# allentran/golds-rl-gym

Hardware: AMD Instinct MI355X
Metric: env-steps/sec (whole node), 32k parallel Swarm-v0 envs, 20-step PAAC rollout (higher is better)
Workload: dtype f32; 1 GPU; Swarm-v0 84x84, 32768 envs per GPU, T=20 PAAC update, conv policy of train_paac_conv.py (BASELINE configs[2]); envs_per_gpu=32768, envs_total=32768, rollout_steps=20, policy=conv, train=True, swarm_math=exact, env_state_dtype=f64, streams=4, gradient_exchange=none

## Files before the change

### golds-rl-gym_amd/csrc/net_conv.hip

```cpp
#include <stdlib.h>
#include <string.h>

#include <chrono>
#include <cmath>
#include <string>
#include <vector>

#include "../../include/goldsrl_net.h"
#include "common.h"
#include "net_gemm.h"
#include "net_paac_host.h"
#include "net_reduce.inc"
#include "rng.h"

namespace grl {

enum : uint32_t { RS_ACTION = 16 };

struct ConvOffsets {
    static constexpr long c1w = 0, c1b = c1w + 8 * 8 * 3 * 32, c2w = c1b + 32, c2b = c2w + 4 * 4 * 32 * 64, c3w = c2b + 64,
                          c3b = c3w + 3 * 3 * 64 * 64, d1w = c3b + 64, d1b = d1w + 3136 * 512, d2w = d1b + 512,
                          d2b = d2w + 512 * 256, p1w = d2b + 256, p1b = p1w + 256 * 512, heads = p1b + 512;
};
constexpr int GRL_MAX_ACTIONS = 4;
// ... 71 lines not shown
    unsigned long long *ws_m2s;
    signed char *ws_ulist;
    void *ws_idx[24];
    bool train_ready;
};

struct NetEval {
    double *rewards, *normals;
    int32_t *length;
    uint8_t *finished, *alive;
    float *envact, *actions;
    float *tr_mu, *tr_sigma, *tr_raw, *tr_value;
    size_t cap_steps, cap_norm, cap_envs, cap_act, cap_trace;
    int max_steps, trace_env, keep_actions;
    bool unchecked;
    int flag_before;
};

struct grl_net : NetLane, grl::PaacCommNet {
    grl_net_config cfg;
    int chunk;
    float *paramsT;
    float *w3t, *w2t;
    float *w3f;
    float *wpvT;
    int shared_trunk;
    double sfrac;
    double pfrac[3];
    float *tbgimg, *tbgz, *tbgimg3, *tbgz3, *tybg;
    int *tbglist;
    int obs_index;
    int trunk_skip;
    int patch_skip;
    int gemm_f32, range_fallback_on, range_fallbacks, range_bits_last, update_skipped_last;
    int f32_by_fallback, f32_clean_passes, range_return_k, range_returns;
    float absmax_last;
    int loss_scale_on;
    int acc1;
    int expand3_gather;
    int expand2_gemm, ctiles;
    float *w2corr;
    grl::HeadOff ho;
    int npad, ptiles, pslices, pslice_rows, pwgrad_xcd, pdgrad_xcd, pwgrad_pair, pdgrad_pair, swgrad_pair, swgrad_chunks, slots_xcd;
    int tn_wgs, tn_wgs_dense;
    size_t slab_floats, slab_used, slabb_floats, slabb_used;
    std::vector<grl::RJob> rq;
    std::vector<int> rq_dst;
    int T, B;
    uint8_t *ro_lb, *ro_ab, *ro_pos, *ro_done;
    float *ro_act, *ro_envact, *ro_val, *ro_rew, *ro_y, *ro_adv, *ro_boot, *ro_pmu, *ro_psg;
    float *mu, *sigma, *vs;
    uint8_t *tmp_lb, *tmp_ab, *tmp_pos;
    int tmp_envs;
    bool prof_on;
    std::vector<hipEvent_t> prof_ev;
    std::vector<unsigned char> prof_tag;
    std::vector<double> prof_launch_flops;
    int prof_tag_cur;
    size_t prof_used;
    double prof_flops;
    int last_n;
    long ht_rollouts, ht_updates;
    double ht_rollout_ms, ht_train_enq_ms, ht_train_wait_ms;
    double ht_train_t0;
    int keep_level;
    float *keep;
// ... 277 lines not shown
        for (int d = 1; d < 32; d <<= 1) {
            const int o = __shfl_up(incl, d, 32);
            if (co >= d) incl += o;
        }
        const int total = __shfl(incl, 31, 32);
        int at = incl - n;
#pragma unroll
        for (int j = 0; j < 4; ++j) {
            const unsigned int k = (w >> (8 * j)) & 255u;
            if (k) ev[at++] = (unsigned short)((((ky * 8 + half * 4 + j) * 2 + c) << 7) | k);
        }
        float acc = b1[co];
        for (int e = 0; e < total; ++e) {
            const int code = ev[e];
            acc += vtab[(code >> 7) & 1][code & 127] * wl[(code >> 7) * 32 + co];
        }
        if (live) sraw[(size_t)env * 12800 + pix * 32 + co] = acc;
    }
    __syncthreads();
    if (tid < 90 && bx != 255) {
        const int idx = bx * G + by;
        cnt[tid < 80 ? 0 : 1][idx >> 2] = 0u;
    }
  }
}

__device__ __forceinline__ float wave_sum(float v) {
#pragma unroll
    for (int o = 32; o > 0; o >>= 1) v += __shfl_xor(v, o);
    return v;
}

constexpr int kHeadRows = 4;
template <int A>
__global__ __launch_bounds__(256) void heads_forward_kernel(const float *__restrict__ p1, const float *__restrict__ v2,
                                                            const float *__restrict__ params, HeadOff o, int n, float scale,
                                                            float *__restrict__ mu, float *__restrict__ sigma, float *__restrict__ vs) {
    const int row0 = (blockIdx.x * 4 + (threadIdx.x >> 6)) * kHeadRows, lane = threadIdx.x & 63;
    if (row0 >= n) return;
    const float *muw = params + o.muw, *sgw = params + o.sgw, *v3w = params + o.v3w;
    float wm[8][A], ws[8][A];
#pragma unroll
    for (int j = 0; j < 8; ++j) {
        const int k = (j >> 2) * 256 + 4 * lane + (j & 3);
#pragma unroll
        for (int a = 0; a < A; ++a) { wm[j][a] = muw[k * A + a]; ws[j][a] = sgw[k * A + a]; }
    }
    const float4 wv = make_float4(v3w[4 * lane], v3w[4 * lane + 1], v3w[4 * lane + 2], v3w[4 * lane + 3]);
    float4 x0[kHeadRows], x1[kHeadRows], xv[kHeadRows];
#pragma unroll
    for (int r = 0; r < kHeadRows; ++r) {
        const size_t row = (size_t)min(row0 + r, n - 1);
        x0[r] = reinterpret_cast<const float4 *>(p1 + row * 512)[lane];
        x1[r] = reinterpret_cast<const float4 *>(p1 + row * 512 + 256)[lane];
        xv[r] = reinterpret_cast<const float4 *>(v2 + row * 256)[lane];
    }
    float mine = 0.f;
#pragma unroll
    for (int r = 0; r < kHeadRows; ++r) {
        const float x[8] = {x0[r].x, x0[r].y, x0[r].z, x0[r].w, x1[r].x, x1[r].y, x1[r].z, x1[r].w};
#pragma unroll
        for (int a = 0; a < A; ++a) {
            float m = 0.f, sg = 0.f;
#pragma unroll
            for (int j = 0; j < 8; ++j) { m += x[j] * wm[j][a]; sg += x[j] * ws[j][a]; }
            m = wave_sum(m);
            sg = wave_sum(sg);
            if (lane == 16 * r + a) mine = m;
            if (lane == 16 * r + A + a) mine = sg;
        }
        const float zv = wave_sum(xv[r].x * wv.x + xv[r].y * wv.y + xv[r].z * wv.z + xv[r].w * wv.w);
        if (lane == 16 * r + 2 * A) mine = zv;
    }
    const int r = lane >> 4, i = lane & 15, row = row0 + r;
    if (row >= n || i > 2 * A) return;
    if (i < A) {
        mu[(size_t)row * A + i] = tanhf(mine + params[o.mub + i]);
    } else if (i < 2 * A) {
        sigma[(size_t)row * A + (i - A)] = 1.0f / (1.0f + expf(-(mine + params[o.sgb + (i - A)])));
    } else {
        const float zv = mine + params[o.v3b];
        const float sp = zv > 20.f ? zv : log1pf(expf(zv));
        vs[row] = -scale * sp;
    }
}
#define GRL_HEADS_DISPATCH(A_, CALL)                                  \
    switch (A_) {                                                     \
        case 1: { constexpr int kA = 1; CALL; } break;                \
        case 2: { constexpr int kA = 2; CALL; } break;                \
        case 3: { constexpr int kA = 3; CALL; } break;                \
        default: { constexpr int kA = 4; CALL; } break;               \
    }

struct ObsRecord {
    const uint32_t *lb, *ab, *pos;
    uint32_t *ro_lb, *ro_ab, *ro_pos;
    int nenv;
    int32_t *done_count;
};
__global__ void sample_actions_kernel(const float *__restrict__ mu, const float *__restrict__ sigma, int i0, int n, uint64_t seed,
                                      uint32_t env_off, uint32_t counter, float *__restrict__ raw, float *__restrict__ envact, ObsRecord R) {
    int i = blockIdx.x * blockDim.x + threadIdx.x;
    if (R.done_count && i == 0) *R.done_count = 0;
    for (int w = i; w < R.nenv * 50; w += gridDim.x * blockDim.x) {
        if (w < R.nenv * 40) R.ro_lb[w] = R.lb[w];
        else if (w < R.nenv * 45) R.ro_ab[w - R.nenv * 40] = R.ab[w - R.nenv * 40];
        else R.ro_pos[w - R.nenv * 45] = R.pos[w - R.nenv * 45];
    }
// ... 56 lines not shown
    if (net->shared_trunk) {
        net->a3sh = b; b += (c / 10) * 3136;
        net->d3 = b; b += c * 1600;
        net->m3 = reinterpret_cast<unsigned long long *>(b); b += c * 50;
    } else {
        net->a3 = b; b += c * 3136;
    }
    net->d1 = b; b += c * 512;
    net->d2 = b; b += c * 256;
    net->p1 = b; b += c * 512;
    net->v1 = b; b += c * 512;
    net->v2 = b; b += c * 256;
    net->mb_d2 = reinterpret_cast<unsigned long long *>(b); net->mb_v1 = net->mb_d2 + c * 4; b += c * 32;
    if (net->shared_trunk && net->keep_level >= 2) {
        net->sraw = b; b += (c / 10) * 12800;
        net->a2sh = b; b += (c / 10) * 5184;
        net->d2s = b; b += c * 576;
        net->m2s = reinterpret_cast<unsigned long long *>(b); b += c * 18;
        net->ulist = reinterpret_cast<signed char *>(b); b += ((c * 9 + 3) / 4 + 3) / 4 * 4;
    }
    size_t walked = (size_t)(b - b0) * sizeof(float);
    if (net->shared_trunk && net->keep_level >= 3) {
        const size_t used = (size_t)(b - b0);
        char *q = reinterpret_cast<char *>(b + (((used + 31) & ~(size_t)31) - used));
#define X(m, bytes) net->m = reinterpret_cast<decltype(net->m)>(q); q += ((size_t)(bytes) + 127) & ~(size_t)127;
        GRL_IDX_LIST(X)
#undef X
        walked = (size_t)(q - reinterpret_cast<char *>(b0));
    }
    return walked;
}

static int forward_chunk(grl_net *net, const uint8_t *lb, const uint8_t *ab, const uint8_t *pos, int nenv, float *mu,
                         float *sigma, float *vs, bool reuse_tail = false, bool skip_heads = false) {
    hipStream_t st = net->h->stream;
    const float *P = net->params, *PT = net->paramsT;
    const int n = nenv * 10;
    net->last_n = n;
    net->pitem_on_side = 0;
    if (net->shared_trunk) {
        int rc;
        if (reuse_tail && net->keep_level >= 3) {
            if ((rc = slot_prof(net, n))) return rc;
            rc = patch_prof(net);
        } else if (reuse_tail && net->keep_level >= 2) {
            if ((rc = slot_index(net, pos, n))) return rc;
            if (net->trunk_skip && net->expand2_gemm && (rc = trunk_index(net, lb, ab, pos, nenv))) return rc;
            rc = patch_sort(net, n);
        } else {
            rc = forward_conv12_shared(net, lb, ab, pos, nenv, !reuse_tail);
        }
        if (rc) return rc;
    } else {
    net->prof_tag_cur = PT_PER_AGENT;
    hipLaunchKernelGGL(conv1_sparse_kernel, dim3(nenv), dim3(256), 0, st, lb, ab, pos, P + ConvOffsets::c1w, P + ConvOffsets::c1b,
                       net->a1, net->h->cfg.grid_size, (float *)nullptr);
    {
        GatherConv2 g{net->a1, n * 81};
        EpiBiasAct e{net->a2, 64, P + ConvOffsets::c2b, ACT_RELU};
        GemmTimer t(net, 2.0 * n * 81 * 512 * 64);
        launch_rowk<256, 64, kW256M, kW256N, GatherConv2, EpiBiasAct>(net, dim3(1, (n * 81 + 255) / 256), st, g, PT + ConvOffsets::c2w, 512, 64, e);
    }
    }
    if (!reuse_tail) {
    if (net->shared_trunk) {
        if (int rc = forward_conv3_dense1_shared(net, nenv, pos)) return rc;
    } else {
        GatherConv3 g{net->a2, n * 49};
        EpiBiasAct e{net->a3, 64, P + ConvOffsets::c3b, ACT_RELU};
        GemmTimer t(net, 2.0 * n * 49 * 576 * 64);
        launch_rowk<256, 64, kW256M, kW256N, GatherConv3, EpiBiasAct>(net, dim3(1, (n * 49 + 255) / 256), st, g, PT + ConvOffsets::c3w, 576, 64, e);
    }
    net->prof_tag_cur = net->shared_trunk ? PT_DENSE_FWD : PT_PER_AGENT;
    auto dense = [&](const float *in, int K, const float *w, const float *b, int N, float *out, unsigned long long *bits) {
        DenseRows g{in, n, K, K};
        GemmTimer t(net, 2.0 * n * K * N);
        if (bits) {
            EpiBiasActBits e{out, N, b, bits, N >> 6};
            launch_rowk<128, 128, kW128M, kW128N, DenseRows, EpiBiasActBits>(net, dim3(N / 128, (n + 127) / 128), st, g, w, K, N, e);
        } else {
            EpiBiasAct e{out, N, b, ACT_RELU};
            launch_rowk<128, 128, kW128M, kW128N, DenseRows, EpiBiasAct>(net, dim3(N / 128, (n + 127) / 128), st, g, w, K, N, e);
        }
    };
    if (!net->shared_trunk) dense(net->a3, 3136, PT + ConvOffsets::d1w, P + ConvOffsets::d1b, 512, net->d1, nullptr);
    dense(net->d1, 512, PT + ConvOffsets::d2w, P + ConvOffsets::d2b, 256, net->d2, net->mb_d2);
    {
        DenseRows g{net->d2, n, 256, 256};
        GemmTimer t(net, 2.0 * n * 256 * 1024);
        EpiBiasActSplit e{net->p1, net->v1, 512, 512, P + ConvOffsets::p1b, P + net->ho.v1b, net->mb_v1, 8};
        launch_rowk<128, 128, kW128M, kW128N, DenseRows, EpiBiasActSplit, true, true, 1, true>(net, dim3(1024 / 128, (n + 127) / 128), st, g, net->wpvT, 256, 1024, e);
    }
    dense(net->v1, 512, PT + net->ho.v2w, P + net->ho.v2b, 256, net->v2, nullptr);
    }
    if (!skip_heads)
    GRL_HEADS_DISPATCH(net->ho.A, hipLaunchKernelGGL(heads_forward_kernel<kA>, dim3((n + 4 * kHeadRows - 1) / (4 * kHeadRows)), dim3(256), 0, st, net->p1, net->v2, P, net->ho, n,
                                                      net->cfg.scale, mu, sigma, vs));
    PAAC_HIP(net, hipGetLastError());
    return GRL_OK;
}

static int forward_all(grl_net *net, const uint8_t *lb, const uint8_t *ab, const uint8_t *pos, int n_envs, float *mu, float *sigma,
                       float *vs, long slot0 = -1) {
    const int ce = net->chunk / 10;
    int rc = lanes_fork(net);
    if (rc) return rc;
    const int nl = lanes_active(net);
    for (int e0 = 0; e0 < n_envs; e0 += ce) {
        int ne = n_envs - e0 < ce ? n_envs - e0 : ce;
        use_lane(net, (e0 / ce) % nl);
        net->last_lane = net->cur_lane;
        bind_activations(net, slot0 < 0 ? -1 : slot0 + e0 / ce);
        rc = forward_chunk(net, lb + (size_t)e0 * 160, ab + (size_t)e0 * 20, pos + (size_t)e0 * 20, ne,
                           mu + (size_t)e0 * 10 * net->ho.A, sigma + (size_t)e0 * 10 * net->ho.A, vs + (size_t)e0 * 10);
        if (rc) { (void)lanes_join(net); return rc; }
    }
    return lanes_join(net);
}

static int alloc_lane_forward(grl_net *n) {
    const size_t c = n->chunk;
    int rc = GRL_OK;
    auto A = [&](float **p, size_t cnt) { if (rc == GRL_OK) rc = paac_alloc(n, p, cnt); };
    A(&n->grads, n->ho.total);
    const size_t gather_ws = (size_t)n->ctiles * 256 * 576 + (c * 25 + 256) * 4 + (c * 25 + 1024) + 2 * ((c + 255) / 256 + 1) * 64 + 4096;
    A(&n->a2, std::max(c * 5184, gather_ws)); A(&n->d1, c * 512); A(&n->d2, c * 256); A(&n->p1, c * 512); A(&n->v1, c * 512); A(&n->v2, c * 256);
    if (!n->shared_trunk) { A(&n->a1, c * 12800); A(&n->a3, c * 3136); }
    A(&n->sraw, (c / 10) * 12800); A(&n->z2sh, (c / 10) * 5184);
    A(&n->a2sh, (c / 10) * 5184); A(&n->d2s, c * 9 * 64); if (rc == GRL_OK) rc = paac_alloc(n, &n->m2s, c * 9); A(&n->z3sh, (c / 10) * 3136);
// ... 172 lines not shown
    grl_net *n = new grl_net();
    n->h = h; n->cfg = *cfg; n->chunk = cfg->max_chunk_samples; n->alloc_waits = true;
    n->ho = head_offsets(cfg->num_actions); n->num_params = n->ho.total;
    n->T = 0; n->B = 0; n->tmp_envs = 0; n->prof_on = false; n->prof_used = 0; n->prof_flops = 0; n->last_n = 0; n->prof_tag_cur = 0;
    n->ro_lb = nullptr; n->slab_floats = 0; n->slab_used = 0; n->slabb_floats = 0; n->slabb_used = 0; n->w3t = n->w2t = nullptr;
    n->mu = n->sigma = n->vs = nullptr;
    n->keep_level = 0;
    n->ht_rollouts = n->ht_updates = 0; n->ht_rollout_ms = n->ht_train_enq_ms = n->ht_train_wait_ms = 0.0; n->ht_train_t0 = 0.0;
    n->keep = nullptr; n->keep_slots = 0; n->param_version = 0; n->keep_version = -1;
    n->keep_max_level = 3; n->keep_free_capped = false; n->keep_free_cap = 0; n->keep_headroom = 0; n->keep_free_seen = 0;
    n->resident_last = 0;
    if (const char *e = getenv("GRL_NET_KEEP_LEVEL")) n->keep_max_level = atoi(e);
    n->keep_free_capped = free_capped; n->keep_free_cap = (size_t)free_mb << 20;
    n->shared_trunk = (cfg->reserved & GRL_NET_F_PER_AGENT_TRUNK) ? 0 : 1;
    n->cur_lane = 0; n->last_lane = 0;
    for (int k = 0; k < GRL_MAX_LANES; ++k) { n->lane_stream[k] = nullptr; n->ev_join[k] = nullptr; n->side_stream[k] = nullptr; n->ev_side0[k] = n->ev_side1[k] = n->ev_side2[k] = nullptr; }
    n->idx_side = 0; n->side_now = 0; n->pitem_on_side = 0;
    n->lane_stream[0] = h->stream; n->ev_fork = nullptr; n->nlanes = 1;
    const size_t c = n->chunk;
    n->ptiles = (int)((c + 255) / 256) + 9;
    n->ctiles = (int)((c + 255) / 256) + 4;
    {
        const char *lsk = getenv("GRL_NET_LOSS_SCALE");
        n->loss_scale_on = (lsk && strcmp(lsk, "off") == 0) ? 0 : 1;
        const char *gm = getenv("GRL_NET_GEMM"), *rf = getenv("GRL_NET_RANGE_FALLBACK");
        n->gemm_f32 = (gm && strcmp(gm, "f32") == 0) ? 1 : 0;
        n->range_fallback_on = (rf && strcmp(rf, "off") == 0) ? 0 : 1;
        n->range_fallbacks = 0; n->range_bits_last = 0; n->update_skipped_last = 0;
        n->f32_by_fallback = 0; n->f32_clean_passes = 0; n->range_returns = 0; n->absmax_last = 0.f;
        n->range_return_k = 4;
        if (const char *rr = getenv("GRL_NET_RANGE_RETURN")) n->range_return_k = strcmp(rr, "off") == 0 ? 0 : std::max(0, atoi(rr));
        const char *psk = getenv("GRL_PATCH_SKIP");
        n->patch_skip = (psk && strcmp(psk, "off") == 0) ? 0 : 1;
        const char *oix = getenv("GRL_OBS_INDEX");
        n->obs_index = (oix && strcmp(oix, "off") == 0) ? 0 : 1;
        const char *tsk = getenv("GRL_TRUNK_SKIP");
        n->trunk_skip = (tsk && strcmp(tsk, "off") == 0) ? 0 : 1;
        n->pfrac[0] = n->pfrac[1] = n->pfrac[2] = 1.0; n->sfrac = 1.0;
        const char *e2 = getenv("GRL_NET_EXPAND2");
        n->expand2_gemm = (e2 && strcmp(e2, "lds") == 0) ? 0 : 1;
        { const char *e3 = getenv("GRL_NET_EXPAND3"); n->expand3_gather = (e3 && strcmp(e3, "prod") == 0) ? 0 : 1;
          const char *a1 = getenv("GRL_NET_ACC1"); n->acc1 = (a1 && strcmp(a1, "off") == 0) ? 0 : 1; }
    }
    n->pslice_rows = PATCH_SLICE_ROWS; n->pwgrad_xcd = 1;
    if (const char *e = getenv("GRL_PATCH_SLICE")) { const int v = atoi(e); if (v == 256 || v == 512 || v == 1024 || v == 2048 || v == 4096 || v == 8192) n->pslice_rows = v; }
    if (const char *e = getenv("GRL_PATCH_WGRAD_XCD")) n->pwgrad_xcd = atoi(e);
    n->pwgrad_pair = 1;
    if (const char *e = getenv("GRL_PATCH_WGRAD_PAIR")) n->pwgrad_pair = strcmp(e, "off") != 0 && strcmp(e, "0") != 0;
    n->pdgrad_pair = 1;
    if (const char *e = getenv("GRL_PATCH_DGRAD_PAIR")) n->pdgrad_pair = strcmp(e, "off") != 0 && strcmp(e, "0") != 0;
    n->swgrad_pair = 1;
    if (const char *e = getenv("GRL_SLOT_WGRAD_PAIR")) n->swgrad_pair = strcmp(e, "off") != 0 && strcmp(e, "0") != 0;
    n->slots_xcd = 1;
    if (const char *e = getenv("GRL_SLOTS_XCD")) n->slots_xcd = strcmp(e, "off") != 0 && strcmp(e, "0") != 0;
    n->swgrad_chunks = 0;
    if (const char *e = getenv("GRL_SLOT_WGRAD_CHUNKS")) n->swgrad_chunks = std::max(0, atoi(e));
    n->pdgrad_xcd = 1;
    n->tn_wgs = 1024; n->tn_wgs_dense = 512;
    if (const char *e = getenv("GRL_TN_WGS")) { const int v = atoi(e); if (v >= 256 && v <= 4096) n->tn_wgs = v; }
    if (const char *e = getenv("GRL_TN_WGS_DENSE")) { const int v = atoi(e); if (v >= 128 && v <= 4096) n->tn_wgs_dense = v; }
    if (const char *e = getenv("GRL_PATCH_DGRAD_XCD")) n->pdgrad_xcd = atoi(e) != 0;
    n->pslices = (int)((c + n->pslice_rows - 1) / n->pslice_rows) + 9;
    n->npad = (int)((c + 255) / 256 * 256);
    int rc = GRL_OK;
    auto A = [&](float **p, size_t cnt) { if (rc == GRL_OK) rc = paac_alloc(n, p, cnt); };
    A(&n->params, n->ho.total); A(&n->paramsT, n->ho.total); A(&n->adam_m, n->ho.total); A(&n->adam_v, n->ho.total);
// ... 392 lines not shown
```

### golds-rl-gym_amd/csrc/net_gemm.h

```cpp
#pragma once
#include <hip/hip_runtime.h>
#include <stdint.h>

#include <type_traits>
#include <utility>

namespace grl {

template <class E, class = void>
struct epi_row_bits : std::false_type {};
template <class E>
struct epi_row_bits<E, std::void_t<decltype(E::kRowBits)>> : std::bool_constant<E::kRowBits> {};

template <class E, class = void>
struct epi_row_auxn : std::false_type {};
template <class E>
struct epi_row_auxn<E, std::void_t<decltype(E::kRowAuxN)>> : std::bool_constant<E::kRowAuxN> {};
template <class E, class = void>
struct epi_add_aux : std::false_type {};
template <class E>
struct epi_add_aux<E, std::void_t<decltype(E::kAddAux)>> : std::bool_constant<E::kAddAux> {};

typedef float f32x16 __attribute__((ext_vector_type(16)));
typedef float f32x4 __attribute__((ext_vector_type(4)));
// ... 192 lines not shown
        off = (long)r * ld;
        iy0 = ix0 = 0;
    }
    __device__ __forceinline__ void tap(int k0, int &toff, int &ty, int &tx) const {
        toff = k0;
        ty = tx = 0;
    }
    __device__ __forceinline__ bool ok(int, int, int, int) const { return true; }
    __device__ __forceinline__ bool tile_ok(int, int) const { return true; }
    __device__ __forceinline__ bool tile_active(int m0) const { return !rows_dev || m0 < *rows_dev; }
    __device__ __forceinline__ int bk(int k0, int) const { return k0; }
    __device__ __forceinline__ int bn(int n0, int) const { return n0; }
    __device__ __forceinline__ int2 ahandle(int m) const { return make_int2(m, 0); }
    __device__ __forceinline__ bool hvalid(int2) const { return true; }
    __device__ __forceinline__ int bhandle(int m) const { return m; }
    __device__ __forceinline__ void rowh(int2 h, long &off, int &iy0, int &ix0) const { row(h.x, off, iy0, ix0); }
    __device__ __forceinline__ void mrange(int z, int mc, int &mbeg, int &mend) const { mbeg = z * mc; mend = min(rows, mbeg + mc); }
};

struct DenseRowsKU : DenseRows {
    static constexpr int kMaxK = 64 * 64;
    const unsigned *u;
    __device__ __forceinline__ unsigned long long wg_ctx(int) const { return (unsigned long long)u[0] | ((unsigned long long)u[1] << 32); }
    __device__ __forceinline__ bool tile_ok_c(unsigned long long c, int k0) const { return (c >> (k0 >> 6)) & 1ull; }
    __device__ __forceinline__ int bk_c(unsigned long long, int k0) const { return k0; }
};
struct DenseRowsNU : DenseRows {
    const unsigned *u;
    __device__ __forceinline__ bool n_ok(int, int n0) const { return (u[n0 >> 11] >> ((n0 >> 6) & 31)) & 1u; }
};
struct DenseRowsIU : DenseRows {
    const unsigned *u;
    __device__ __forceinline__ bool i_ok(int, int i0) const { return (u[i0 >> 11] >> ((i0 >> 6) & 31)) & 1u; }
};

struct DenseRowsGroups {
    static constexpr bool kRelu = false;
    const float *base;
    int rows, ld, k, npad, nlive, bnstep, cpc;
    __device__ __forceinline__ int K() const { return k; }
    __device__ __forceinline__ void row(int r, long &off, int &iy0, int &ix0) const {
        off = (long)r * ld;
        iy0 = ix0 = 0;
    }
    __device__ __forceinline__ void tap(int k0, int &toff, int &ty, int &tx) const {
        toff = k0;
        ty = tx = 0;
    }
    __device__ __forceinline__ bool ok(int, int, int, int) const { return true; }
    __device__ __forceinline__ bool tile_ok(int, int) const { return true; }
    __device__ __forceinline__ bool tile_active(int m0) const { return m0 % npad < nlive; }
    __device__ __forceinline__ int bk(int k0, int) const { return k0; }
    __device__ __forceinline__ int bn(int n0, int m0) const { return n0 + (m0 / npad) * bnstep; }
    __device__ __forceinline__ int2 ahandle(int m) const { return make_int2(m, 0); }
    __device__ __forceinline__ bool hvalid(int2) const { return true; }
    __device__ __forceinline__ int bhandle(int m) const { return m; }
    __device__ __forceinline__ void rowh(int2 h, long &off, int &iy0, int &ix0) const { row(h.x, off, iy0, ix0); }
    __device__ __forceinline__ void mrange(int z, int mc, int &mbeg, int &mend) const {
        const int g = z / cpc, c = z - g * cpc;
        mbeg = g * npad + c * mc;
        mend = min(g * npad + nlive, mbeg + mc);
    }
};

struct T2SlotGather {
    static constexpr bool kRelu = false;
// ... 630 lines not shown
        b0[b] = *reinterpret_cast<const float4 *>(Bf + f32_off(brow + b * 16, 8 * kg));
        b1[b] = *reinterpret_cast<const float4 *>(Bf + f32_off(brow + b * 16, 8 * kg + 4));
    }
#define GRL_F32_STEP(AV, BV)                                                                                          \
    _Pragma("unroll") for (int a = 0; a < TM; ++a)                                                                    \
        _Pragma("unroll") for (int b = 0; b < TN; ++b) acc[a][b] = __builtin_amdgcn_mfma_f32_16x16x4f32(AV, BV, acc[a][b], 0, 0, 0);
    GRL_F32_STEP(a0[a].x, b0[b].x) GRL_F32_STEP(a0[a].y, b0[b].y) GRL_F32_STEP(a0[a].z, b0[b].z) GRL_F32_STEP(a0[a].w, b0[b].w)
    GRL_F32_STEP(a1[a].x, b1[b].x) GRL_F32_STEP(a1[a].y, b1[b].y) GRL_F32_STEP(a1[a].z, b1[b].z) GRL_F32_STEP(a1[a].w, b1[b].w)
#undef GRL_F32_STEP
}

template <class T, class = void> struct ag_has_ctx : std::false_type {};
template <class T> struct ag_has_ctx<T, std::void_t<decltype(std::declval<const T &>().wg_ctx(0))>> : std::true_type {};
template <class AG> __device__ __forceinline__ auto ag_ctx(const AG &ag, int m0) {
    if constexpr (ag_has_ctx<AG>::value) return ag.wg_ctx(m0);
    else return m0;
}
template <class AG, class C> __device__ __forceinline__ bool ag_tile_ok(const AG &ag, const C &c, int m0, int k0) {
    if constexpr (ag_has_ctx<AG>::value) return ag.tile_ok_c(c, k0);
    else return ag.tile_ok(m0, k0);
}
template <class AG, class C> __device__ __forceinline__ int ag_bk(const AG &ag, const C &c, int m0, int k0) {
    if constexpr (ag_has_ctx<AG>::value) return ag.bk_c(c, k0);
    else return ag.bk(k0, m0);
}
template <class T, class = void> struct ag_has_n_ok : std::false_type {};
template <class T> struct ag_has_n_ok<T, std::void_t<decltype(std::declval<const T &>().n_ok(0, 0))>> : std::true_type {};
template <class T, class = void> struct ag_has_i_ok : std::false_type {};
template <class T> struct ag_has_i_ok<T, std::void_t<decltype(std::declval<const T &>().i_ok(0, 0))>> : std::true_type {};
template <class T, class = void> struct ag_pair_n : std::false_type {};
template <class T> struct ag_pair_n<T, std::void_t<decltype(T::kPairN)>> : std::bool_constant<T::kPairN> {};
template <class T, class = void> struct ag_pair_i : std::false_type {};
template <class T> struct ag_pair_i<T, std::void_t<decltype(T::kPairI)>> : std::bool_constant<T::kPairI> {};

template <int BM, int BN, int WGM, int WGN, class AG, class Epi, int XCD_ORDER = 1, bool FENCE = true, bool F32 = false, int NBUF = 1, bool ACC1 = false>
__global__ __launch_bounds__(64 * WGM * WGN, ACC1 ? (WGM * WGN == 8 ? 6 : 4) : WGM * WGN / 2) void gemm_rowk(AG ag, const float *__restrict__ Bt, int ldb, int N, Epi epi) {
    constexpr int BK = 32, LDH = kLdh, NT = 64 * WGM * WGN, RPP = NT / 8;
    constexpr int WM = BM / WGM, WN = BN / WGN, TM = WM / 16, TN = WN / 16;
    constexpr int NA = BM / RPP;
    constexpr int NB = BN / RPP;
    static_assert((WGM * WGN == 4 || WGM * WGN == 8) && TM >= 1 && TN >= 1 && NA >= 1 && BN % RPP == 0, "4 or 8 waves");
    static_assert(NBUF == 1 || NBUF == 2, "one or two LDS buffers");
    __shared__ __attribute__((aligned(16))) unsigned short As[NBUF][2][BM * LDH];
    static_assert(!(ACC1 && F32), "the fp32 form has one accumulator set anyway");
    __shared__ __attribute__((aligned(16))) unsigned short Bs[NBUF][ACC1 ? 3 : 2][BN * LDH];

    const int tid = threadIdx.x, lane = tid & 63, wave = tid >> 6;
    const int wm = wave / WGN, wn = wave - wm * WGN;
    int bx = blockIdx.x, by = blockIdx.y;
    if constexpr (XCD_ORDER == 2) {
        const int nt = (ag.live_rows() + BM - 1) / BM, tpx = (nt + 7) >> 3, w = blockIdx.y;
        if ((w >> 3) >= tpx) return;
        by = (w & 7) * tpx + (w >> 3);
        if (by >= nt) return;
    }
    if (XCD_ORDER == 1) {
        const int nx = gridDim.x, L = by * nx + bx, g = L / (8 * nx);
        if ((g + 1) * 8 <= (int)gridDim.y) {
            const int l = L - g * 8 * nx;
            by = g * 8 + (l & 7);
            bx = l >> 3;
        }
    }
    const int m0 = by * BM, n0 = bx * BN;
    if (!ag.tile_active(m0)) return;
    constexpr bool PAIRN = ag_pair_n<AG>::value;
// ... 242 lines not shown
            for (int a = 0; a < TM; ++a)
#pragma unroll
                for (int r = 0; r < 4; ++r)
                    if (erow + a * 16 + r < M) sum += epi.value(acc[a][b][r], eax[a][b][r]);
            sum += __shfl_xor(sum, 16);
            sum += __shfl_xor(sum, 32);
            const int col = ecol + b * 16;
            if (kg == 0 && col < N) epi.csum[(long)(by * WGM + wm) * N + col] = sum;
        }
    }
    if constexpr (epi_row_bits<Epi>::value) {
        static_assert(WN == 64, "a wave covers exactly one 64-column block");
#pragma unroll
        for (int a = 0; a < TM; ++a)
#pragma unroll
            for (int r = 0; r < 4; ++r) {
                unsigned long long w = 0ull;
#pragma unroll
                for (int b = 0; b < TN; ++b) {
                    const unsigned long long bal = __ballot(epi.bit(acc[a][b][r], eax[a][b][r]));
                    w |= ((bal >> (16 * kg)) & 0xFFFFull) << (16 * b);
                }
                const int row = erow + a * 16 + r;
                if (l16 == 0 && row < M) epi.store_bits(row, ecolbase, w, rax[a][r]);
            }
    }
#undef GRL_LOAD_TILE
#undef GRL_STORE_TILE
#undef GRL_STORE_PLANES
#undef GRL_STORE_PLANES_B
}

template <int BM, int BN, int WGM, int WGN, class AG, int XCD_ORDER = 1, bool F32 = false>
__global__ __launch_bounds__(64 * WGM * WGN, WGM * WGN / 2) void gemm_tn(AG ag, const float *__restrict__ dY, int J, int mc, float *__restrict__ slab) {
    constexpr int BK = 32, LDH = kLdh, NT = 64 * WGM * WGN;
    constexpr int WM = BM / WGM, WN = BN / WGN, TM = WM / 16, TN = WN / 16;
    constexpr int A4 = BM / 4, B4 = BN / 4;
    constexpr int NA = BK * A4 / NT, NB = BK * B4 / NT;
    static_assert((WGM * WGN == 4 || WGM * WGN == 8) && NA >= 1 && NB >= 1 && NA <= 4 && NB <= 4 && (NA != 3) && (NB != 3), "tile size");
    __shared__ __attribute__((aligned(16))) unsigned short As[2][BM * LDH];
    __shared__ __attribute__((aligned(16))) unsigned short Bs[2][BN * LDH];
    const int tid = threadIdx.x, lane = tid & 63, wave = tid >> 6;
    const int wm = wave / WGN, wn = wave - wm * WGN;
    int bx = blockIdx.x, by = blockIdx.y, bz = blockIdx.z;
    if (XCD_ORDER == 2) {
        const int nx = gridDim.x, ny = gridDim.y, l = by * nx + bx, g = l / (8 * ny);
        if ((g + 1) * 8 <= nx) {
            const int r = l - g * 8 * ny;
            bx = g * 8 + (r & 7);
            by = r >> 3;
        } else {
            const int r = l - g * 8 * ny, w = nx - g * 8;
            by = r / w;
            bx = g * 8 + (r - by * w);
        }
    }
    if (XCD_ORDER == 1) {
        const int nx = gridDim.x, T = nx * gridDim.y, L = bz * T + by * nx + bx, g = L / (8 * T);
        if ((g + 1) * 8 <= (int)gridDim.z) {
            const int l = L - g * 8 * T, t = l >> 3;
            bz = g * 8 + (l & 7);
            by = t / nx;
            bx = t - by * nx;
        }
    }
    constexpr bool PAIR = ag_pair_i<AG>::value;
    const int i0 = bx * BM, j0 = by * BN;
    const int I = ag.K();
    int mbeg, mend;
    ag.mrange(bz, mc, mbeg, mend);
    int2 pp = make_int2(0, 0);
    if constexpr (PAIR) {
        static_assert(!PAIR || BM == 128, "two 64-column halves");
        pp = ag.pair(bz, bx);
        if (pp.x < 0) return;
    } else if constexpr (ag_has_i_ok<AG>::value) {
        if (!ag.i_ok(bz, i0)) return;
    }

    int toff, ty, tx;
    ag.tap(PAIR ? (((int)(threadIdx.x % (BM / 4)) < 16 ? pp.x : max(pp.y, 0)) * 64) : i0, toff, ty, tx);

    const int ca = tid % A4, cb = tid % B4;
    int ga = tid / A4, gb = tid / B4;
    if (NA == 4) ga ^= (ca >> 1) & 1;
    if (NA == 2) ga ^= ((ca >> 1) & 1) << 1;
    if (NB == 4) gb ^= (cb >> 1) & 1;
    if (NB == 2) gb ^= ((cb >> 1) & 1) << 1;
    if (NB == 1) gb ^= ((cb >> 1) & 1) << 2;
    const int ma = NA * ga, mb = NB * gb;
    const int acol = PAIR ? toff + (ca & 15) * 4 : toff + ca * 4;
    const bool ahalf_ok = !PAIR || ca < 16 || pp.y >= 0;
    float4 ra[NA], rb[NB];
    unsigned vma = 0, vmb = 0;
    int2 ia[NA];
    int ib[NB];
    unsigned iva = 0;
#define GRL_LOAD_IDX(mt_)                                                                                          \
    {                                                                                                              \
        _Pragma("unroll") for (int i = 0; i < NA; ++i) {                                                           \
// ... 239 lines not shown
```

### golds-rl-gym_amd/csrc/net_slab_plan.h

```cpp
#pragma once
#include <stddef.h>

namespace grl {

struct SlabPlan {
    int chunks;
    int mc;
};

inline SlabPlan slab_plan(int wg_target, int tiles, int min_chunks, int rows, size_t floats_per_chunk, size_t slab_floats) {
    int chunks = (wg_target + tiles - 1) / tiles;
    if (min_chunks > chunks) chunks = min_chunks;
    if (chunks > 1024) chunks = 1024;
    if ((size_t)chunks * floats_per_chunk > slab_floats) chunks = (int)(slab_floats / floats_per_chunk);
    if (chunks < 1 || rows == 0) return {chunks, 0};
    const int mc = ((rows + chunks - 1) / chunks + 31) / 32 * 32;
    return {(rows + mc - 1) / mc, mc};
}

}
```

### golds-rl-gym_amd/csrc/net_train.inc

```

#include "net_slab_plan.h"

namespace grl {

static inline double host_now_ms() {
    return std::chrono::duration<double, std::milli>(std::chrono::steady_clock::now().time_since_epoch()).count();
}

static int rq_flush(grl_net *net) {
    const int nj = (int)net->rq.size();
    if (!nj) { net->slab_used = 0; net->slabb_used = 0; return GRL_OK; }
    std::vector<int> phase(nj, 0);
    int maxph = 0;
    for (int k = 0; k < nj; ++k) {
        for (int i = 0; i < k; ++i) phase[k] += net->rq_dst[i] == net->rq_dst[k];
        maxph = std::max(maxph, phase[k]);
    }
    for (int ph = 0; ph <= maxph; ++ph) {
        int k = 0;
        while (k < nj) {
            RBatch B;
            B.njobs = 0;
            int blocks = 0;
            for (; k < nj && B.njobs < kRJobs; ++k) {
// ... 892 lines not shown
    }
    return GRL_OK;
}

static int bwd_conv2_dgrad(const BwdCtx &c) {
    const auto [net, st, P, Gr, n, nenv, trunk] = c;
    net->prof_tag_cur = PT_ENV_DGRAD;
    float *cs5 = slabb_take(net, ((size_t)nenv * 100 / 128 + 2) * kW128M * 128);
    if (!cs5) return paac_fail(net, GRL_E_INVALID, "backward_chunk: column-sum buffer too small");
    if (trunk) {
        rowk_launch<128, 128, 2, 2, false>(net, GatherT2Rows{net->dz2, net->tblklist, net->trows_n + 1, nenv * 100}, net->w2t, 256, 128,
                                    EpiGradStride2Rows{net->gt, net->sraw, cs5, P + ConvOffsets::c1b, net->tblklist, net->trows_n + 1},
                                    2.0 * trunk_live(net, 1, (double)nenv * 100) * 256 * 128);
        hipLaunchKernelGGL(fold_class_sums_kernel, dim3(kFoldParts), dim3(256), 0, st, cs5, (nenv * 100 + 127) / 128 * 2, net->cfold,
                           (const int *)(net->trows_n + 1));
    } else {
        rowk_launch<128, 128, 2, 2, false>(net, GatherT2{net->dz2, nenv * 100}, net->w2t, 256, 128,
                                    EpiGradStride2<true, true>{net->gt, net->sraw, cs5}, 2.0 * nenv * 100 * 256 * 128);
        hipLaunchKernelGGL(fold_class_sums_kernel, dim3(kFoldParts), dim3(256), 0, st, cs5, (nenv * 100 + 127) / 128 * 2, net->cfold,
                           (const int *)nullptr);
    }
    {
        RJob j{};
        j.kind = RJ_FOLDFINAL; j.blocks = 1; j.p0 = net->cfold; j.d0 = Gr + ConvOffsets::c1b;
        rq_push(net, RD_C1B, j);
    }
    return GRL_OK;
}

static int bwd_dense_wgrad(const BwdCtx &c) {
    const auto [net, st, P, Gr, n, nenv, trunk] = c;
    int rc;
    if ((rc = tn_launch<128, 128, 2, 2>(net, RD_V2W, DenseRows{net->v1, n, 512, 512}, 512, net->gv2, 256, Gr + net->ho.v2w, 1, 0.0, 0, net->tn_wgs_dense))) return rc;
    if ((rc = tn_launch<128, 128, 2, 2>(net, RD_V1W, DenseRows{net->d2, n, 256, 256}, 256, net->gv1, 512, Gr + net->ho.v1w, 1, 0.0, 0, net->tn_wgs_dense))) return rc;
    if ((rc = tn_launch<128, 128, 2, 2>(net, RD_P1W, DenseRows{net->d2, n, 256, 256}, 256, net->gp1, 512, Gr + ConvOffsets::p1w, 1, 0.0, 0, net->tn_wgs_dense))) return rc;
    if ((rc = tn_launch<128, 128, 2, 2>(net, RD_D2W, DenseRows{net->d1, n, 512, 512}, 512, net->gd2, 256, Gr + ConvOffsets::d2w, 1, 0.0, 0, net->tn_wgs_dense))) return rc;
    return GRL_OK;
}

static int bwd_dense1_wgrad(const BwdCtx &c) {
    const auto [net, st, P, Gr, n, nenv, trunk] = c;
    int rc;
    net->prof_tag_cur = PT_ENV_WGRAD;
    if (trunk) {
        constexpr int I = 3136, J = 512;
        int chunks, mc;
        float *slab = slab_plan_take(net, net->tn_wgs, (I / 64) * (J / 128), 0, nenv, (size_t)I * J, "dense1 per-env weight gradient: slab too small", &chunks, &mc);
        if (!slab) return GRL_E_INVALID;
        {
            GemmTimer t(net, 2.0 * nenv * 64.0 * trunk_union_pixels(net) * J);
            launch_tn<64, 128, 2, 2, DenseRowsIU>(net, dim3(I / 64, J / 128, chunks), st, DenseRowsIU{{net->a3sh, nenv, 3136, 3136}, net->tumask},
                                                  net->gd1sh, J, mc, slab);
        }
        RJob j{};
        j.kind = RJ_UMASK; j.blocks = (int)(((long)I * J + 255) / 256); j.i0 = chunks; j.n = (long)I * J; j.p0 = slab; j.p1 = net->tumask;
        j.p2 = net->tbgz3 + 64; j.p3 = net->tug; j.d0 = Gr + ConvOffsets::d1w;
        rq_push(net, RD_D1W, j);
    } else if ((rc = tn_launch<64, 128, 2, 2>(net, RD_D1W, DenseRows{net->a3sh, nenv, 3136, 3136}, 3136, net->gd1sh, 512, Gr + ConvOffsets::d1w))) return rc;
    {
        float *pslab = slab_take(net, (size_t)net->pslices * 1600 * 512);
        if (!pslab) return paac_fail(net, GRL_E_INVALID, "backward_chunk: slab too small for the patch slices");
        PatchRows g{net->d3, net->perm, net->tilegroup, net->ptiles * 256, 1600, 1600, 0, net->sbeg, net->send, net->patch_skip ? net->tmask : nullptr,
                    net->patch_skip ? net->zmask : nullptr};
        {
            net->prof_tag_cur = PT_PATCH_WGRAD;
            GemmTimer t(net, 2.0 * n * 1600 * 512 * net->pfrac[2]);
            if (net->pwgrad_pair) {
                PatchRowsPair gp{g};
// ... 347 lines not shown
}

using namespace grl;

extern "C" {

int grl_net_rollout(grl_net *net, int32_t T, int32_t reward_layout) {
    if (!net || T <= 0 || T > 1024 || (reward_layout != 0 && reward_layout != 1)) return paac_fail(net, GRL_E_INVALID, "grl_net_rollout: bad argument");
    const double ht0 = host_now_ms();
    grl_handle *h = net->h;
    if (net->ho.A != 2) return paac_fail(net, GRL_E_INVALID, "grl_net_rollout: SwarmEnv.step takes (10, 2) actions; this net was built with num_actions != 2");
    hipSetDevice(h->cfg.device_id);
    int rc = ensure_rollout_bufs(net, T);
    if (rc) return rc;
    const int E = h->E, B = E * 10, ce = net->chunk / 10, nchunks = (E + ce - 1) / ce;
    net->T = T;
    net->keep_version = net->keep && (size_t)T * nchunks <= net->keep_slots ? net->param_version : -1;
    if (reward_layout == 1) PAAC_HIP(net, hipMemsetAsync(net->ro_rew, 0, (size_t)T * B * 4, h->stream));
    if ((rc = lanes_fork(net))) return rc;
    const int nl = lanes_active(net);
    net->side_now = nchunks == 1;
    struct SideOff { grl_net *n; ~SideOff() { n->side_now = 0; } } side_off{net};
    const unsigned long counter0 = net->act_counter;
    net->act_counter += (unsigned long)T;
    for (int t = 0; t <= T; ++t)
        for (int c = 0; c < nchunks; ++c) {
            const int e0 = c * ce, ne = E - e0 < ce ? E - e0 : ce;
            use_lane(net, c % nl);
            net->last_lane = net->cur_lane;
            hipStream_t st = h->stream;
            if (t == T) {
                bind_activations(net, -1);
                rc = forward_chunk(net, h->sw.lbins + (size_t)e0 * 160, h->sw.abins + (size_t)e0 * 20, h->sw.pos + (size_t)e0 * 20, ne,
                                   net->mu + (size_t)e0 * 20, net->sigma + (size_t)e0 * 20, net->ro_boot + (size_t)e0 * 10);
                if (rc) { (void)lanes_join(net); return rc; }
                continue;
            }
            bind_activations(net, net->keep_version >= 0 ? (long)t * nchunks + c : -1);
            rc = forward_chunk(net, h->sw.lbins + (size_t)e0 * 160, h->sw.abins + (size_t)e0 * 20, h->sw.pos + (size_t)e0 * 20, ne,
                               net->ro_pmu + ((size_t)t * B + (size_t)e0 * 10) * 2, net->ro_psg + ((size_t)t * B + (size_t)e0 * 10) * 2,
                               net->ro_val + (size_t)t * B + (size_t)e0 * 10);
            if (rc) { (void)lanes_join(net); return rc; }
            ObsRecord rec{reinterpret_cast<const uint32_t *>(h->sw.lbins + (size_t)e0 * 160), reinterpret_cast<const uint32_t *>(h->sw.abins + (size_t)e0 * 20),
                          reinterpret_cast<const uint32_t *>(h->sw.pos + (size_t)e0 * 20),
                          reinterpret_cast<uint32_t *>(net->ro_lb + ((size_t)t * E + e0) * 160), reinterpret_cast<uint32_t *>(net->ro_ab + ((size_t)t * E + e0) * 20),
                          reinterpret_cast<uint32_t *>(net->ro_pos + ((size_t)t * E + e0) * 20), ne, h->done_count + net->cur_lane};
            hipLaunchKernelGGL(sample_actions_kernel, dim3((ne * 10 + 255) / 256), dim3(256), 0, st, net->ro_pmu + (size_t)t * B * 2,
                               net->ro_psg + (size_t)t * B * 2, e0 * 10, ne * 10, h->cfg.seed,
                               (uint32_t)h->cfg.env_id_offset, (uint32_t)(counter0 + (unsigned long)t), net->ro_act + (size_t)t * B * 2, net->ro_envact, rec);
            if ((rc = swarm_launch_step_range(h, net->ro_envact, e0, ne, net->cur_lane, true)) ||
                (rc = episodes_launch_account(h, e0, ne))) {
                (void)lanes_join(net);
                return paac_fail(net, rc, h->err);
            }
            hipLaunchKernelGGL(reward_layout_kernel, dim3((ne * 10 + 255) / 256), dim3(256), 0, st, h->reward, e0, ne, reward_layout,
                               net->ro_rew + (size_t)t * B, (const uint8_t *)h->done, net->ro_done + (size_t)t * E);
        }
    if ((rc = lanes_join(net))) return rc;
    if ((rc = launch_returns(h, net->ro_rew, net->ro_val, nullptr, net->ro_boot, T, B, net->cfg.gamma, 1.0f, net->cfg.scale, 0.f, 0.f,
                             net->ro_y, net->ro_adv)))
        return paac_fail(net, rc, h->err);
    hipLaunchKernelGGL(rollout_range_mark_kernel, dim3(1), dim3(1), 0, h->stream, range_flag_ptr(net));
    PAAC_HIP(net, hipGetLastError());
    h->step_in_flight = true;
    net->ht_rollout_ms += host_now_ms() - ht0;
    net->ht_rollouts += 1;
    return GRL_OK;
// ... 206 lines not shown
```

Baseline: 2.309 million env-steps/s.

## Skip policy head on bootstrap forward and merge v1/p1 weight-gradient launches

For the bootstrap forward at step T, only the value head is computed: the dense p1/v1 GEMM drops the policy half and the heads kernel skips the mu/sigma math and stores. In the backward pass, the v1 and p1 weight-gradient TN GEMMs, which share the same input d2, become one launch with a split-J grid, and the per-target slab reductions are queued separately. Together these cut GEMM work and a kernel launch, at the cost of extra slab memory and a new code path gated by GRL_DENSE_BITS. Bootstrap mu/sigma buffers are no longer written on that step.

```diff
diff --git a/golds-rl-gym_amd/csrc/net_conv.hip b/golds-rl-gym_amd/csrc/net_conv.hip
--- a/golds-rl-gym_amd/csrc/net_conv.hip
+++ b/golds-rl-gym_amd/csrc/net_conv.hip
@@ -127,6 +127,7 @@
     int obs_index;
     int trunk_skip;
     int patch_skip;
+    int dense_bits;
     int gemm_f32, range_fallback_on, range_fallbacks, range_bits_last, update_skipped_last;
     int f32_by_fallback, f32_clean_passes, range_return_k, range_returns;
     float absmax_last;
@@ -470,7 +471,7 @@
 }
 
 constexpr int kHeadRows = 4;
-template <int A>
+template <int A, bool VONLY = false>
 __global__ __launch_bounds__(256) void heads_forward_kernel(const float *__restrict__ p1, const float *__restrict__ v2,
                                                             const float *__restrict__ params, HeadOff o, int n, float scale,
                                                             float *__restrict__ mu, float *__restrict__ sigma, float *__restrict__ vs) {
@@ -478,24 +479,29 @@
     if (row0 >= n) return;
     const float *muw = params + o.muw, *sgw = params + o.sgw, *v3w = params + o.v3w;
     float wm[8][A], ws[8][A];
+    if constexpr (!VONLY) {
 #pragma unroll
     for (int j = 0; j < 8; ++j) {
         const int k = (j >> 2) * 256 + 4 * lane + (j & 3);
 #pragma unroll
         for (int a = 0; a < A; ++a) { wm[j][a] = muw[k * A + a]; ws[j][a] = sgw[k * A + a]; }
     }
+    }
     const float4 wv = make_float4(v3w[4 * lane], v3w[4 * lane + 1], v3w[4 * lane + 2], v3w[4 * lane + 3]);
     float4 x0[kHeadRows], x1[kHeadRows], xv[kHeadRows];
 #pragma unroll
     for (int r = 0; r < kHeadRows; ++r) {
         const size_t row = (size_t)min(row0 + r, n - 1);
+        if constexpr (!VONLY) {
         x0[r] = reinterpret_cast<const float4 *>(p1 + row * 512)[lane];
         x1[r] = reinterpret_cast<const float4 *>(p1 + row * 512 + 256)[lane];
+        }
         xv[r] = reinterpret_cast<const float4 *>(v2 + row * 256)[lane];
     }
     float mine = 0.f;
 #pragma unroll
     for (int r = 0; r < kHeadRows; ++r) {
+        if constexpr (!VONLY) {
         const float x[8] = {x0[r].x, x0[r].y, x0[r].z, x0[r].w, x1[r].x, x1[r].y, x1[r].z, x1[r].w};
 #pragma unroll
         for (int a = 0; a < A; ++a) {
@@ -507,11 +513,12 @@
             if (lane == 16 * r + a) mine = m;
             if (lane == 16 * r + A + a) mine = sg;
         }
+        }
         const float zv = wave_sum(xv[r].x * wv.x + xv[r].y * wv.y + xv[r].z * wv.z + xv[r].w * wv.w);
         if (lane == 16 * r + 2 * A) mine = zv;
     }
     const int r = lane >> 4, i = lane & 15, row = row0 + r;
-    if (row >= n || i > 2 * A) return;
+    if (row >= n || i > 2 * A || (VONLY && i < 2 * A)) return;
     if (i < A) {
         mu[(size_t)row * A + i] = tanhf(mine + params[o.mub + i]);
     } else if (i < 2 * A) {
@@ -634,7 +641,7 @@
 }
 
 static int forward_chunk(grl_net *net, const uint8_t *lb, const uint8_t *ab, const uint8_t *pos, int nenv, float *mu,
-                         float *sigma, float *vs, bool reuse_tail = false, bool skip_heads = false) {
+                         float *sigma, float *vs, bool reuse_tail = false, bool skip_heads = false, bool value_only = false) {
     hipStream_t st = net->h->stream;
     const float *P = net->params, *PT = net->paramsT;
     const int n = nenv * 10;
@@ -687,7 +694,12 @@
     };
     if (!net->shared_trunk) dense(net->a3, 3136, PT + ConvOffsets::d1w, P + ConvOffsets::d1b, 512, net->d1, nullptr);
     dense(net->d1, 512, PT + ConvOffsets::d2w, P + ConvOffsets::d2b, 256, net->d2, net->mb_d2);
-    {
+    if (value_only) {
+        DenseRows g{net->d2, n, 256, 256};
+        GemmTimer t(net, 2.0 * n * 256 * 512);
+        EpiBiasActSplit e{nullptr, net->v1, 512, 0, nullptr, P + net->ho.v1b, net->mb_v1, 8};
+        launch_rowk<128, 128, kW128M, kW128N, DenseRows, EpiBiasActSplit, true, true, 1, true>(net, dim3(512 / 128, (n + 127) / 128), st, g, net->wpvT + (size_t)512 * 256, 256, 512, e);
+    } else {
         DenseRows g{net->d2, n, 256, 256};
         GemmTimer t(net, 2.0 * n * 256 * 1024);
         EpiBiasActSplit e{net->p1, net->v1, 512, 512, P + ConvOffsets::p1b, P + net->ho.v1b, net->mb_v1, 8};
@@ -695,8 +707,11 @@
     }
     dense(net->v1, 512, PT + net->ho.v2w, P + net->ho.v2b, 256, net->v2, nullptr);
     }
-    if (!skip_heads)
-    GRL_HEADS_DISPATCH(net->ho.A, hipLaunchKernelGGL(heads_forward_kernel<kA>, dim3((n + 4 * kHeadRows - 1) / (4 * kHeadRows)), dim3(256), 0, st, net->p1, net->v2, P, net->ho, n,
+    if (!skip_heads && value_only) {
+    GRL_HEADS_DISPATCH(net->ho.A, hipLaunchKernelGGL((heads_forward_kernel<kA, true>), dim3((n + 4 * kHeadRows - 1) / (4 * kHeadRows)), dim3(256), 0, st, net->p1, net->v2, P, net->ho, n,
+                                                      net->cfg.scale, mu, sigma, vs));
+    } else if (!skip_heads)
+    GRL_HEADS_DISPATCH(net->ho.A, hipLaunchKernelGGL((heads_forward_kernel<kA, false>), dim3((n + 4 * kHeadRows - 1) / (4 * kHeadRows)), dim3(256), 0, st, net->p1, net->v2, P, net->ho, n,
                                                       net->cfg.scale, mu, sigma, vs));
     PAAC_HIP(net, hipGetLastError());
     return GRL_OK;
@@ -935,6 +950,8 @@
         if (const char *rr = getenv("GRL_NET_RANGE_RETURN")) n->range_return_k = strcmp(rr, "off") == 0 ? 0 : std::max(0, atoi(rr));
         const char *psk = getenv("GRL_PATCH_SKIP");
         n->patch_skip = (psk && strcmp(psk, "off") == 0) ? 0 : 1;
+        const char *dbt = getenv("GRL_DENSE_BITS");
+        n->dense_bits = (dbt && strcmp(dbt, "off") == 0) ? 0 : 1;
         const char *oix = getenv("GRL_OBS_INDEX");
         n->obs_index = (oix && strcmp(oix, "off") == 0) ? 0 : 1;
         const char *tsk = getenv("GRL_TRUNK_SKIP");
diff --git a/golds-rl-gym_amd/csrc/net_gemm.h b/golds-rl-gym_amd/csrc/net_gemm.h
--- a/golds-rl-gym_amd/csrc/net_gemm.h
+++ b/golds-rl-gym_amd/csrc/net_gemm.h
@@ -248,6 +248,11 @@
 struct DenseRowsIU : DenseRows {
     const unsigned *u;
     __device__ __forceinline__ bool i_ok(int, int i0) const { return (u[i0 >> 11] >> ((i0 >> 6) & 31)) & 1u; }
+};
+struct DenseRowsSplitJ : DenseRows {
+    static constexpr bool kSplitJ = true;
+    const float *dY2;
+    float *slab2;
 };
 
 struct DenseRowsGroups {
@@ -944,6 +949,8 @@
 template <class T> struct ag_pair_n<T, std::void_t<decltype(T::kPairN)>> : std::bool_constant<T::kPairN> {};
 template <class T, class = void> struct ag_pair_i : std::false_type {};
 template <class T> struct ag_pair_i<T, std::void_t<decltype(T::kPairI)>> : std::bool_constant<T::kPairI> {};
+template <class T, class = void> struct ag_split_j : std::false_type {};
+template <class T> struct ag_split_j<T, std::void_t<decltype(T::kSplitJ)>> : std::bool_constant<T::kSplitJ> {};
 
 template <int BM, int BN, int WGM, int WGN, class AG, class Epi, int XCD_ORDER = 1, bool FENCE = true, bool F32 = false, int NBUF = 1, bool ACC1 = false>
 __global__ __launch_bounds__(64 * WGM * WGN, ACC1 ? (WGM * WGN == 8 ? 6 : 4) : WGM * WGN / 2) void gemm_rowk(AG ag, const float *__restrict__ Bt, int ldb, int N, Epi epi) {
@@ -1252,8 +1259,10 @@
 }
 
 template <int BM, int BN, int WGM, int WGN, class AG, int XCD_ORDER = 1, bool F32 = false>
-__global__ __launch_bounds__(64 * WGM * WGN, WGM * WGN / 2) void gemm_tn(AG ag, const float *__restrict__ dY, int J, int mc, float *__restrict__ slab) {
+__global__ __launch_bounds__(64 * WGM * WGN, WGM * WGN / 2) void gemm_tn(AG ag, const float *__restrict__ dY0, int J, int mc, float *__restrict__ slab0) {
     constexpr int BK = 32, LDH = kLdh, NT = 64 * WGM * WGN;
+    const float *dY = dY0;
+    float *slab = slab0;
     constexpr int WM = BM / WGM, WN = BN / WGN, TM = WM / 16, TN = WN / 16;
     constexpr int A4 = BM / 4, B4 = BN / 4;
     constexpr int NA = BK * A4 / NT, NB = BK * B4 / NT;
@@ -1285,7 +1294,11 @@
         }
     }
     constexpr bool PAIR = ag_pair_i<AG>::value;
-    const int i0 = bx * BM, j0 = by * BN;
+    const int i0 = bx * BM;
+    int j0 = by * BN;
+    if constexpr (ag_split_j<AG>::value) {
+        if (j0 >= J) { j0 -= J; dY = ag.dY2; slab = ag.slab2; }
+    }
     const int I = ag.K();
     int mbeg, mend;
     ag.mrange(bz, mc, mbeg, mend);
diff --git a/golds-rl-gym_amd/csrc/net_slab_plan.h b/golds-rl-gym_amd/csrc/net_slab_plan.h
--- a/golds-rl-gym_amd/csrc/net_slab_plan.h
+++ b/golds-rl-gym_amd/csrc/net_slab_plan.h
@@ -18,4 +18,16 @@
     return {(rows + mc - 1) / mc, mc};
 }
 
+struct SlabPlanPair {
+    SlabPlan each;
+    bool merged;
+};
+inline SlabPlanPair slab_plan_pair(int wg_target, int tiles_each, int min_chunks, int rows, size_t floats_per_chunk, size_t slab_floats,
+                                   size_t slab_used) {
+    const SlabPlan p = slab_plan(wg_target, tiles_each, min_chunks, rows, floats_per_chunk, slab_floats);
+    if (p.chunks < 1) return {p, false};
+    const size_t one = ((size_t)p.chunks * floats_per_chunk + 63) & ~(size_t)63;
+    return {p, slab_used + 2 * one <= slab_floats};
 }
+
+}
diff --git a/golds-rl-gym_amd/csrc/net_train.inc b/golds-rl-gym_amd/csrc/net_train.inc
--- a/golds-rl-gym_amd/csrc/net_train.inc
+++ b/golds-rl-gym_amd/csrc/net_train.inc
@@ -948,8 +948,31 @@
     const auto [net, st, P, Gr, n, nenv, trunk] = c;
     int rc;
     if ((rc = tn_launch<128, 128, 2, 2>(net, RD_V2W, DenseRows{net->v1, n, 512, 512}, 512, net->gv2, 256, Gr + net->ho.v2w, 1, 0.0, 0, net->tn_wgs_dense))) return rc;
+    constexpr int I = 256, J = 512;
+    const SlabPlanPair pp = slab_plan_pair(net->tn_wgs_dense, (I / 128) * (J / 128), 0, n, (size_t)I * J, slab_left(net), net->slab_used);
+    if (net->dense_bits && pp.merged) {
+        int chv, chp, mcv, mcp;
+        float *slabv = slab_plan_take(net, net->tn_wgs_dense, (I / 128) * (J / 128), 0, n, (size_t)I * J, "tn_launch: slab too small", &chv, &mcv);
+        if (!slabv) return GRL_E_INVALID;
+        float *slabp = slab_plan_take(net, net->tn_wgs_dense, (I / 128) * (J / 128), 0, n, (size_t)I * J, "tn_launch: slab too small", &chp, &mcp);
+        if (!slabp) return GRL_E_INVALID;
+        if (chv != pp.each.chunks || chp != chv || mcv != pp.each.mc || mcp != mcv || net->rq.empty())
+            return paac_fail(net, GRL_E_INVALID, "bwd_dense_wgrad: the two plans of the merged launch disagree");
+        {
+            GemmTimer t(net, 2.0 * (double)n * I * (2 * J));
+            launch_tn<128, 128, 2, 2, DenseRowsSplitJ>(net, dim3(I / 128, 2 * J / 128, chp), st, DenseRowsSplitJ{{net->d2, n, 256, 256}, net->gv1, slabv},
+                                                       net->gp1, J, mcp, slabp);
+        }
+        RJob j{};
+        j.kind = RJ_SLAB; j.blocks = (I * J + 255) / 256; j.i0 = chv; j.i1 = 1; j.n = (long)I * J; j.p0 = slabv; j.d0 = Gr + net->ho.v1w;
+        rq_push(net, RD_V1W, j);
+        j.p0 = slabp; j.d0 = Gr + ConvOffsets::p1w;
+        rq_push(net, RD_P1W, j);
+        PAAC_HIP(net, hipGetLastError());
+    } else {
     if ((rc = tn_launch<128, 128, 2, 2>(net, RD_V1W, DenseRows{net->d2, n, 256, 256}, 256, net->gv1, 512, Gr + net->ho.v1w, 1, 0.0, 0, net->tn_wgs_dense))) return rc;
     if ((rc = tn_launch<128, 128, 2, 2>(net, RD_P1W, DenseRows{net->d2, n, 256, 256}, 256, net->gp1, 512, Gr + ConvOffsets::p1w, 1, 0.0, 0, net->tn_wgs_dense))) return rc;
+    }
     if ((rc = tn_launch<128, 128, 2, 2>(net, RD_D2W, DenseRows{net->d1, n, 512, 512}, 512, net->gd2, 256, Gr + ConvOffsets::d2w, 1, 0.0, 0, net->tn_wgs_dense))) return rc;
     return GRL_OK;
 }
@@ -1363,7 +1386,8 @@
             if (t == T) {
                 bind_activations(net, -1);
                 rc = forward_chunk(net, h->sw.lbins + (size_t)e0 * 160, h->sw.abins + (size_t)e0 * 20, h->sw.pos + (size_t)e0 * 20, ne,
-                                   net->mu + (size_t)e0 * 20, net->sigma + (size_t)e0 * 20, net->ro_boot + (size_t)e0 * 10);
+                                   net->mu + (size_t)e0 * 20, net->sigma + (size_t)e0 * 20, net->ro_boot + (size_t)e0 * 10, false, false,
+                                   net->dense_bits != 0);
                 if (rc) { (void)lanes_join(net); return rc; }
                 continue;
             }
```

Result: slower. 2.270 million env-steps/s (-1.7%).
